# templeblock/llzlab

Hardware: AMD Instinct MI355X
Metric: Msamples/s/GPU (float32 FIR 257-tap, 4096 ch) + achieved HBM GB/s vs peak (higher is better)
Workload: dtype f32; 1 GPU; 4096-ch float32 FIR, 257 taps (llz_fir_lpf_cof 0.1 KAISER), 1048576 samples/ch per GPU, overlap-save-1024, channels sharded over 1 GPU(s); channels_per_gpu=4096, samples_per_channel=1048576, taps=257, algorithm=overlap-save-1024

## Files before the change

### llzlab_amd/csrc/kernels/fft32.hpp

```cpp
#pragma once
#include "common.hpp"

namespace {

struct cf {
    float x, y;
};

__device__ __forceinline__ cf cadd(cf a, cf b) { return {a.x + b.x, a.y + b.y}; }
__device__ __forceinline__ cf csub(cf a, cf b) { return {a.x - b.x, a.y - b.y}; }

template <bool CONJ>
__device__ __forceinline__ cf cmul(cf a, cf w)
{
    if (CONJ) return {__builtin_fmaf(a.y, w.y, a.x * w.x), __builtin_fmaf(-a.x, w.y, a.y * w.x)};
    return {__builtin_fmaf(-a.y, w.y, a.x * w.x), __builtin_fmaf(a.x, w.y, a.y * w.x)};
}

__device__ constexpr float kCos32[9] = {1.0f, 0.98078528040323044913f, 0.92387953251128675613f,
                                        0.83146961230254523708f, 0.70710678118654752440f,
                                        0.55557023301960222474f, 0.38268343236508977173f,
                                        0.19509032201612826785f, 0.0f};

template <bool INV>
__device__ __forceinline__ cf tw32(cf d, int q)
{
    if (q == 0) return d;
    if (q == 8) return INV ? cf{-d.y, d.x} : cf{d.y, -d.x};
    constexpr float r = 0.70710678118654752440f;
    if (q == 4) return INV ? cf{(d.x - d.y) * r, (d.x + d.y) * r} : cf{(d.x + d.y) * r, (d.y - d.x) * r};
    if (q == 12) return INV ? cf{-(d.x + d.y) * r, (d.x - d.y) * r} : cf{(d.y - d.x) * r, -(d.x + d.y) * r};
    const float c = q <= 8 ? kCos32[q] : -kCos32[16 - q];
    const float s = q <= 8 ? kCos32[8 - q] : kCos32[q - 8];
    return cmul<!INV>(d, cf{c, s});
}

__device__ constexpr int brev5(int r)
{
    return ((r & 1) << 4) | ((r & 2) << 2) | (r & 4) | ((r & 8) >> 2) | ((r & 16) >> 4);
}

#ifndef LLZ_OLS_DIT
#define LLZ_OLS_DIT 1
#endif

#if !LLZ_OLS_DIT
template <bool INV>
__device__ __forceinline__ void fft32(cf (&v)[32])
{
#pragma unroll
    for (int span = 32; span >= 2; span >>= 1) {
        const int half = span >> 1;
        const int tstep = 32 / span;
#pragma unroll
        for (int blk = 0; blk < 32; blk += span) {
#pragma unroll
            for (int q = 0; q < half; q++) {
                const cf a = v[blk + q], b = v[blk + q + half];
                v[blk + q] = cadd(a, b);
                v[blk + q + half] = tw32<INV>(csub(a, b), q * tstep);
            }
        }
    }
}
#else
template <bool INV>
__device__ __forceinline__ void bfly_dit(cf &a, cf &b, int q)
{
    const cf A = a, B = b;
    if (q == 0) {
        a = cadd(A, B); b = csub(A, B);
        return;
    }
    if (q == 8) {
        const cf wb = INV ? cf{-B.y, B.x} : cf{B.y, -B.x};
        a = cadd(A, wb); b = csub(A, wb);
        return;
    }
    const float c = q <= 8 ? kCos32[q] : -kCos32[16 - q];
    const float s0 = q <= 8 ? kCos32[8 - q] : kCos32[q - 8];
    const float s = INV ? s0 : -s0;
    float p, g, f;
    if (c >= s0 || -c >= s0) {
        const float t = s / c;
        p = __builtin_fmaf(-t, B.y, B.x);
        g = __builtin_fmaf(t, B.x, B.y);
        f = c;
    } else {
        const float r = c / s;
        p = __builtin_fmaf(-r, B.x, B.y);
        g = __builtin_fmaf(r, B.y, B.x);
        a = cf{__builtin_fmaf(-s, p, A.x), __builtin_fmaf(s, g, A.y)};
        b = cf{__builtin_fmaf(s, p, A.x), __builtin_fmaf(-s, g, A.y)};
        return;
    }
    a = cf{__builtin_fmaf(f, p, A.x), __builtin_fmaf(f, g, A.y)};
    b = cf{__builtin_fmaf(-f, p, A.x), __builtin_fmaf(-f, g, A.y)};
}

template <bool INV>
__device__ __forceinline__ void fft32(cf (&v)[32])
{
    cf w[32];
#pragma unroll
    for (int i = 0; i < 32; i++) w[i] = v[brev5(i)];
#pragma unroll
    for (int half = 1; half <= 16; half <<= 1) {
        const int tstep = 16 / half;
#pragma unroll
        for (int blk = 0; blk < 32; blk += 2 * half) {
#pragma unroll
            for (int q = 0; q < half; q++) bfly_dit<INV>(w[blk + q], w[blk + q + half], q * tstep);
        }
    }
#pragma unroll
    for (int r = 0; r < 32; r++) v[r] = w[brev5(r)];
}
#endif

constexpr int OLS_PITCH = 33;
constexpr int OLS_XBUF = 32 * OLS_PITCH;
__device__ __forceinline__ int xaddr(int row, int col) { return row * OLS_PITCH + col; }

#define OLS_WAVE_SYNC() asm volatile("s_waitcnt lgkmcnt(0)" ::: "memory")

template <bool INV>
__device__ __forceinline__ void transpose_twiddle(cf (&v)[32], float *buf, const float2 *__restrict__ tw, int wcol, int rrow)
{
#pragma unroll
    for (int r = 0; r < 32; r++) {
        const float2 w = tw[brev5(r) * 32 + wcol];
        v[r] = cmul<INV>(v[r], cf{w.x, w.y});
    }
#pragma unroll
    for (int r = 0; r < 32; r++) buf[xaddr(brev5(r), wcol)] = v[r].x;
    OLS_WAVE_SYNC();
#pragma unroll
    for (int cidx = 0; cidx < 32; cidx++) v[cidx].x = buf[xaddr(rrow, cidx)];
    OLS_WAVE_SYNC();
#pragma unroll
    for (int r = 0; r < 32; r++) buf[xaddr(brev5(r), wcol)] = v[r].y;
    OLS_WAVE_SYNC();
#pragma unroll
    for (int cidx = 0; cidx < 32; cidx++) v[cidx].y = buf[xaddr(rrow, cidx)];
    OLS_WAVE_SYNC();
}

template <bool INV>
__device__ __forceinline__ void transpose_twiddle(cf (&v)[32], float *buf, const float2 *__restrict__ tw, int l5)
{
    transpose_twiddle<INV>(v, buf, tw, l5, l5);
}

__device__ __forceinline__ void swap32(float &x, float &y)
{
    const auto p = __builtin_amdgcn_permlane32_swap(__float_as_uint(x), __float_as_uint(y), false, false);
    x = __uint_as_float(p[0]);
    y = __uint_as_float(p[1]);
}

}
```

### llzlab_amd/csrc/kernels/fir_ols.hip

```cpp
#include <stdlib.h>
#include "common.hpp"
#include "fft32.hpp"

namespace {

constexpr int OLS_N = 1024;
constexpr int OLS_OVERLAP = 256;
constexpr int OLS_VALID = OLS_N - OLS_OVERLAP;
constexpr int OLS_JOB = 2 * OLS_VALID;
constexpr int OLS_WAVES = 4;
constexpr int OLS_THREADS = 64 * OLS_WAVES;
constexpr int OLS_SEG = 16;

struct ols_lane {
    int half, col;
};

__device__ __forceinline__ ols_lane ols_lane_of(int lane)
{
    ols_lane g;
    g.half = lane >> 5;
    g.col = lane & 31;
    return g;
}

struct ols_seg {
    bool live;
    int c, j0, count;
};

struct ols_geom {
    int n, keep, jobs_per_channel, segs_per_channel, seg_len;
    long total_segs, in_pitch, out_pitch;
};

__device__ __forceinline__ ols_seg ols_locate(long seg, const ols_geom &G)
{
    ols_seg g;
    g.live = seg < G.total_segs;
    g.c = g.live ? (int)(seg / G.segs_per_channel) : 0;
    g.j0 = g.live ? (int)(seg - (long)g.c * G.segs_per_channel) * G.seg_len : 0;
    g.count = g.live ? min(G.seg_len, G.jobs_per_channel - g.j0) : 0;
    return g;
}

struct ols_raw {
    float a[24], b[24];
};

__device__ __forceinline__ void ols_load(ols_raw &raw, const float *const (&row)[2], const int (&s)[2],
                                         const bool (&live)[2], const ols_lane &g, int n)
{
    const bool whole = live[0] && live[1] && s[0] + OLS_JOB <= n && s[1] + OLS_JOB <= n;
    const float *r = g.half ? row[1] : row[0];
    const int so = g.half ? s[1] : s[0];
    const bool lv = g.half ? live[1] : live[0];
    if (whole) {
#pragma unroll
        for (int i = 0; i < 24; i++) {
            raw.a[i] = __builtin_nontemporal_load(&r[so + 32 * i + g.col]);
            raw.b[i] = __builtin_nontemporal_load(&r[so + OLS_VALID + 32 * i + g.col]);
        }
    } else {
#pragma unroll
        for (int i = 0; i < 24; i++) {
            const int ia = so + 32 * i + g.col, ib = ia + OLS_VALID;
            const float xa = r[min(ia, n - 1)], xb = r[min(ib, n - 1)];
            raw.a[i] = (lv && ia < n) ? xa : 0.f;
            raw.b[i] = (lv && ib < n) ? xb : 0.f;
        }
    }
}

__device__ __forceinline__ void ols_load_halo(float (&halo)[8], const float *row, const float *hrow, int s, int col,
                                              int keep, bool live)
{
#pragma unroll
    for (int i = 0; i < 8; i++) {
        const int idx = s - OLS_OVERLAP + 32 * i + col;
        float v = 0.f;
        if (live) {
            if (idx >= 0) v = row[idx];
            else if (hrow && idx >= -keep) v = hrow[keep + idx];
        }
        halo[i] = v;
    }
}

__device__ __forceinline__ void ols_filter(cf (&v)[32], cf (&u)[32], float *buf, const float2 *s_tw,
                                           const float2 *s_h, int l5, int col)
{
    fft32<false>(v);
    transpose_twiddle<false>(v, buf, s_tw, col, l5);
    fft32<false>(v);
#pragma unroll
    for (int r = 0; r < 32; r++) {
        const float2 h = s_h[l5 + 32 * brev5(r)];
        u[brev5(r)] = cmul<false>(v[r], cf{h.x, h.y});
    }
    fft32<true>(u);
    transpose_twiddle<true>(u, buf, s_tw, l5, col);
    fft32<true>(u);
}

__device__ __forceinline__ void ols_store(const cf (&u)[32], float *const (&orow)[2], const int (&s)[2],
                                          const bool (&live)[2], const ols_lane &g, int n)
{
    const bool whole = live[0] && live[1] && s[0] + OLS_JOB <= n && s[1] + OLS_JOB <= n;
    const bool lv = g.half ? live[1] : live[0];
    if (!lv) return;
    float *o = g.half ? orow[1] : orow[0];
    const int so = g.half ? s[1] : s[0];
    const int oa = so + g.col - OLS_OVERLAP;
    const int ob = oa + OLS_VALID;
    if (whole) {
#pragma unroll
        for (int r = 0; r < 32; r++) {
            const int n1 = brev5(r);
            if (n1 >= 8) {
                __builtin_nontemporal_store(u[r].x, &o[oa + 32 * n1]);
                __builtin_nontemporal_store(u[r].y, &o[ob + 32 * n1]);
            }
        }
    } else {
#pragma unroll
        for (int r = 0; r < 32; r++) {
            const int n1 = brev5(r);
            if (n1 >= 8) {
                if (oa + 32 * n1 < n) o[oa + 32 * n1] = u[r].x;
                if (ob + 32 * n1 < n) o[ob + 32 * n1] = u[r].y;
            }
        }
    }
}

__device__ __forceinline__ void ols_assemble(cf (&v)[32], float (&halo)[8], const ols_raw &raw)
{
#pragma unroll
    for (int i = 0; i < 8; i++) {
        v[i].x = halo[i];
        v[i].y = raw.a[16 + i];
        halo[i] = raw.b[16 + i];
    }
#pragma unroll
    for (int i = 0; i < 24; i++) {
        v[8 + i].x = raw.a[i];
        v[8 + i].y = raw.b[i];
    }
}

struct ols_smem {
    float2 *tw, *h;
    float *buf;
};

__device__ __forceinline__ ols_smem ols_tables(char *smem, const float2 *__restrict__ hfreq, const float2 *__restrict__ twid)
{
    ols_smem m;
    m.tw = reinterpret_cast<float2 *>(smem);
    m.h = m.tw + 1024;
    for (int i = threadIdx.x; i < 1024; i += OLS_THREADS) {
        m.tw[i] = twid[i];
        m.h[i] = hfreq[i];
    }
    __syncthreads();
    const int wave = threadIdx.x >> 6, half = (threadIdx.x >> 5) & 1;
    m.buf = reinterpret_cast<float *>(m.h + 1024) + (wave * 2 + half) * OLS_XBUF;
    return m;
}

__global__ void __launch_bounds__(OLS_THREADS, 2)
k_fir_ols_chain_f32(const float *__restrict__ in, float *__restrict__ out, const float *__restrict__ hist,
                    const float2 *__restrict__ hfreq, const float2 *__restrict__ twid, ols_geom G)
{
    extern __shared__ __attribute__((aligned(16))) char smem[];
    const ols_smem S = ols_tables(smem, hfreq, twid);
    const int lane = threadIdx.x & 63;
    const int wave = __builtin_amdgcn_readfirstlane(threadIdx.x >> 6);
    const int l5 = lane & 31;
    const ols_lane g = ols_lane_of(lane);
    const long halves_total = (long)gridDim.x * OLS_WAVES * 2;
    const long first = ((long)blockIdx.x * OLS_WAVES + wave) * 2;

    ols_seg cur[2] = {ols_locate(first, G), ols_locate(first + 1, G)};
    float halo[8];
    ols_raw raw;
    {
        const float *const row[2] = {in + (size_t)cur[0].c * G.in_pitch, in + (size_t)cur[1].c * G.in_pitch};
        const ols_seg own = g.half ? cur[1] : cur[0];
        ols_load_halo(halo, g.half ? row[1] : row[0], hist ? hist + (size_t)own.c * G.keep : nullptr, own.j0 * OLS_JOB,
                      g.col, G.keep, own.live);
        const int s0[2] = {cur[0].j0 * OLS_JOB, cur[1].j0 * OLS_JOB};
        const bool lv[2] = {cur[0].count > 0, cur[1].count > 0};
        ols_load(raw, row, s0, lv, g, G.n);
    }
    for (long sp = first; sp < G.total_segs; sp += halves_total) {
        const ols_seg nxt[2] = {ols_locate(sp + halves_total, G), ols_locate(sp + halves_total + 1, G)};
        const float *const row[2] = {in + (size_t)cur[0].c * G.in_pitch, in + (size_t)cur[1].c * G.in_pitch};
        float *const orow[2] = {out + (size_t)cur[0].c * G.out_pitch, out + (size_t)cur[1].c * G.out_pitch};
        const float *const nrow[2] = {in + (size_t)nxt[0].c * G.in_pitch, in + (size_t)nxt[1].c * G.in_pitch};
        const ols_seg nown = g.half ? nxt[1] : nxt[0];
        float halo_n[8];
#pragma unroll
        for (int i = 0; i < 8; i++) halo_n[i] = 0.f;

        const int jmax = max(cur[0].count, cur[1].count);
#pragma unroll 1
        for (int jj = 0; jj < jmax; jj++) {
            const int s[2] = {(cur[0].j0 + jj) * OLS_JOB, (cur[1].j0 + jj) * OLS_JOB};
            const bool live[2] = {jj < cur[0].count, jj < cur[1].count};
            cf v[32], u[32];
            ols_assemble(v, halo, raw);
            const bool in_pair = jj + 1 < jmax;
            {
                const float *const lrow[2] = {in_pair ? row[0] : nrow[0], in_pair ? row[1] : nrow[1]};
                const int sn[2] = {in_pair ? s[0] + OLS_JOB : nxt[0].j0 * OLS_JOB,
                                   in_pair ? s[1] + OLS_JOB : nxt[1].j0 * OLS_JOB};
                const bool ln[2] = {in_pair ? jj + 1 < cur[0].count : nxt[0].count > 0,
                                    in_pair ? jj + 1 < cur[1].count : nxt[1].count > 0};
                ols_load(raw, lrow, sn, ln, g, G.n);
            }
            if (!in_pair)
                ols_load_halo(halo_n, g.half ? nrow[1] : nrow[0], hist ? hist + (size_t)nown.c * G.keep : nullptr,
                              nown.j0 * OLS_JOB, g.col, G.keep, nown.live);
            ols_filter(v, u, S.buf, S.tw, S.h, l5, g.col);
            ols_store(u, orow, s, live, g, G.n);
        }
        cur[0] = nxt[0];
        cur[1] = nxt[1];
#pragma unroll
        for (int i = 0; i < 8; i++) halo[i] = halo_n[i];
    }
}



template <int O>
__global__ void __launch_bounds__(OLS_THREADS, 2)
k_fir_ols2k_chain_f32(const float *__restrict__ in, float *__restrict__ out, const float *__restrict__ hist,
                     const float2 *__restrict__ hfreq2 ,
                     const float2 *__restrict__ twid , const float2 *__restrict__ tw2k ,
                     ols_geom G)
{
    extern __shared__ __attribute__((aligned(16))) char smem[];
    float2 *s_tw = reinterpret_cast<float2 *>(smem);
    float2 *s_h = s_tw + 1024;
    float2 *s_w = s_h + 2048;
    for (int i = threadIdx.x; i < 1024; i += OLS_THREADS) {
        s_tw[i] = twid[i];
        s_h[i] = hfreq2[i];
        s_h[1024 + i] = hfreq2[1024 + i];
        s_w[i] = tw2k[i];
    }
    __syncthreads();
    constexpr int O2K_OVERLAP = O, O2K_VALID = 2048 - O, O2K_JOB = 2 * O2K_VALID;
    constexpr int HP = O / 64, NEW = 32 - HP;
    const int lane = threadIdx.x & 63;
    const int wave = __builtin_amdgcn_readfirstlane(threadIdx.x >> 6);
    const int half = lane >> 5, l5 = lane & 31;
    float *buf = reinterpret_cast<float *>(s_w + 1024) + (wave * 2 + half) * OLS_XBUF;
    const float2 *my_h = s_h + half * 1024;
    const long waves_total = (long)gridDim.x * OLS_WAVES;
    const int rowoff = 32 * half + l5;

    struct segd { const float *row; float *orow; const float *hrow; int j0, count; };
    auto locate = [&](long seg) {
        segd d;
        const bool live = seg < G.total_segs;
        const int c = live ? (int)(seg / G.segs_per_channel) : 0;
        d.j0 = live ? (int)(seg - (long)c * G.segs_per_channel) * G.seg_len : 0;
        d.count = live ? min(G.seg_len, G.jobs_per_channel - d.j0) : 0;
        d.row = in + (size_t)c * G.in_pitch;
        d.orow = out + (size_t)c * G.out_pitch;
        d.hrow = hist ? hist + (size_t)c * G.keep : nullptr;
        return d;
    };
    const int n = G.n;
    auto load_halo = [&](float (&halo)[HP], const segd &d) {
#pragma unroll
        for (int i = 0; i < HP; i++) {
            const int idx = d.j0 * O2K_JOB - O2K_OVERLAP + 64 * i + rowoff;
            float v = 0.f;
            if (d.count > 0) {
                if (idx >= 0) v = d.row[idx];
                else if (d.hrow && idx >= -G.keep) v = d.hrow[G.keep + idx];
            }
            halo[i] = v;
        }
    };
    ols_raw raw;
    auto load = [&](const float *row, int s, bool live) {
        if (live && s + O2K_JOB <= n) {
#pragma unroll
            for (int i = 0; i < NEW; i++) {
                raw.a[i] = __builtin_nontemporal_load(&row[s + 64 * i + rowoff]);
                raw.b[i] = __builtin_nontemporal_load(&row[s + O2K_VALID + 64 * i + rowoff]);
            }
        } else {
#pragma unroll
            for (int i = 0; i < NEW; i++) {
                const int ia = s + 64 * i + rowoff, ib = ia + O2K_VALID;
                const float xa = row[min(ia, n - 1)], xb = row[min(ib, n - 1)];
                raw.a[i] = (live && ia < n) ? xa : 0.f;
                raw.b[i] = (live && ib < n) ? xb : 0.f;
            }
        }
    };

    long seg = (long)blockIdx.x * OLS_WAVES + wave;
    segd cur = locate(seg);
    float halo[HP];
    load_halo(halo, cur);
    load(cur.row, cur.j0 * O2K_JOB, cur.count > 0);
    for (; seg < G.total_segs; seg += waves_total) {
        const segd nxt = locate(seg + waves_total);
        float halo_n[HP];
#pragma unroll
        for (int i = 0; i < HP; i++) halo_n[i] = 0.f;
#pragma unroll 1
        for (int jj = 0; jj < cur.count; jj++) {
            const int s = (cur.j0 + jj) * O2K_JOB;
            const float *row = cur.row;
            float *orow = cur.orow;
            cf v[32], u[32];
#pragma unroll
            for (int i = 0; i < HP; i++) {
                v[i].x = halo[i];
                v[i].y = raw.a[NEW - HP + i];
                halo[i] = raw.b[NEW - HP + i];
            }
#pragma unroll
            for (int i = 0; i < NEW; i++) {
                v[HP + i].x = raw.a[i];
                v[HP + i].y = raw.b[i];
            }
            const bool in_seg = jj + 1 < cur.count;
            load(in_seg ? row : nxt.row, in_seg ? s + O2K_JOB : nxt.j0 * O2K_JOB, in_seg || nxt.count > 0);
            if (!in_seg) load_halo(halo_n, nxt);
            cf w[32];
#pragma unroll
            for (int p = 0; p < 16; p++) {
                cf sm = cadd(v[p], v[p + 16]);
                const float2 t = s_w[64 * p + rowoff];
                cf df = cmul<false>(csub(v[p], v[p + 16]), cf{t.x, t.y});
                swap32(sm.x, df.x);
                swap32(sm.y, df.y);
                w[2 * p] = sm;
                w[2 * p + 1] = df;
            }
            ols_filter(w, u, buf, s_tw, my_h, l5, l5);
            const bool whole = s + O2K_JOB <= n;
            const int oa = s - O2K_OVERLAP + rowoff, ob = oa + O2K_VALID;
#pragma unroll
            for (int p = 0; p < 16; p++) {
                cf P = u[brev5(2 * p)], Q = u[brev5(2 * p + 1)];
                swap32(P.x, Q.x);
                swap32(P.y, Q.y);
                const float2 t = s_w[64 * p + rowoff];
                Q = cmul<true>(Q, cf{t.x, t.y});
                const cf y0 = cadd(P, Q), y1 = csub(P, Q);
                if (whole) {
                    if (p >= HP) {
                        __builtin_nontemporal_store(y0.x, &orow[oa + 64 * p]);
                        __builtin_nontemporal_store(y0.y, &orow[ob + 64 * p]);
                    }
                    __builtin_nontemporal_store(y1.x, &orow[oa + 64 * (p + 16)]);
                    __builtin_nontemporal_store(y1.y, &orow[ob + 64 * (p + 16)]);
                } else {
                    if (p >= HP) {
                        if (oa + 64 * p < n) orow[oa + 64 * p] = y0.x;
                        if (ob + 64 * p < n) orow[ob + 64 * p] = y0.y;
                    }
                    if (oa + 64 * (p + 16) < n) orow[oa + 64 * (p + 16)] = y1.x;
                    if (ob + 64 * (p + 16) < n) orow[ob + 64 * (p + 16)] = y1.y;
                }
            }
        }
        cur = nxt;
#pragma unroll
        for (int i = 0; i < HP; i++) halo[i] = halo_n[i];
    }
}


__device__ __forceinline__ int o8k_lane()
{
    int l = (int)__builtin_amdgcn_mbcnt_hi(~0u, __builtin_amdgcn_mbcnt_lo(~0u, 0u));
    asm volatile("" : "+v"(l));
    return l;
}
constexpr int O4K_WAVES = 8, O4K_THREADS = 64 * O4K_WAVES;

template <int WS = 1>
__device__ __forceinline__ void ols2k_core(cf (&v)[32], cf (&y)[32], float *buf, const float2 *s_tw, const float2 *my_h,
                                           const float2 *s_w, int l5, int rowoff)
{
    cf w[32], u[32];
#pragma unroll
    for (int p = 0; p < 16; p++) {
        cf sm = cadd(v[p], v[p + 16]);
        const float2 t = s_w[WS * (64 * p + rowoff)];
        cf df = cmul<false>(csub(v[p], v[p + 16]), cf{t.x, t.y});
        swap32(sm.x, df.x);
        swap32(sm.y, df.y);
        w[2 * p] = sm;
        w[2 * p + 1] = df;
    }
    ols_filter(w, u, buf, s_tw, my_h, l5, l5);
#pragma unroll
    for (int p = 0; p < 16; p++) {
        cf P = u[brev5(2 * p)], Q = u[brev5(2 * p + 1)];
        swap32(P.x, Q.x);
        swap32(P.y, Q.y);
        const float2 t = s_w[WS * (64 * p + rowoff)];
        Q = cmul<true>(Q, cf{t.x, t.y});
        y[p] = cadd(P, Q);
        y[p + 16] = csub(P, Q);
    }
}

template <int O>
__global__ void __launch_bounds__(O4K_THREADS, 2)
k_fir_ols4k_f32(const float *__restrict__ in, float *__restrict__ out, const float *__restrict__ hist,
                const float2 *__restrict__ hfreq4 , const float2 *__restrict__ twid ,
                const float2 *__restrict__ tw2k , const float2 *__restrict__ tw4k ,
                ols_geom G)
{
    constexpr int V = 4096 - O, JOB = 2 * V, PO = O / 64, PV = V / 64;
    extern __shared__ __attribute__((aligned(16))) char smem[];
    float2 *s_tw = reinterpret_cast<float2 *>(smem);
    float2 *s_w2 = s_tw + 1024;
    float2 *s_w4 = s_w2 + 1024;
    float2 *s_h = s_w4 + 2048;
    for (int i = threadIdx.x; i < 1024; i += O4K_THREADS) {
        s_tw[i] = twid[i];
        s_w2[i] = tw2k[i];
        s_w4[i] = tw4k[i];
        s_w4[1024 + i] = tw4k[1024 + i];
#pragma unroll
        for (int j = 0; j < 4; j++) s_h[1024 * j + i] = hfreq4[1024 * j + i];
    }
    __syncthreads();
    const int wave = __builtin_amdgcn_readfirstlane(threadIdx.x >> 6);
    float *s_buf = reinterpret_cast<float *>(s_h + 4096);
    const long waves_total = (long)gridDim.x * O4K_WAVES;
    const int n = G.n;

    for (long seg = (long)blockIdx.x * O4K_WAVES + wave; seg < G.total_segs; seg += waves_total) {
        const int c = (int)(seg / G.segs_per_channel);
        const int j0 = (int)(seg - (long)c * G.segs_per_channel) * G.seg_len;
        const int count = min(G.seg_len, G.jobs_per_channel - j0);
        const float *row = in + (size_t)c * G.in_pitch;
        float *orow = out + (size_t)c * G.out_pitch;
        const float *hrow = hist ? hist + (size_t)c * G.keep : nullptr;
#pragma unroll 1
        for (int jj = 0; jj < count; jj++) {
            const int s = (j0 + jj) * JOB;
            cf v[64];
            const bool whole = s >= O && s + JOB <= n;
            {
            const int rowoff = o8k_lane();
            if (whole) {
#pragma unroll
                for (int i = 0; i < PO; i++) v[i].x = row[s - O + 64 * i + rowoff];
#pragma unroll
                for (int i = PO; i < 64; i++) v[i].x = __builtin_nontemporal_load(&row[s - O + 64 * i + rowoff]);
#pragma unroll
                for (int i = PO; i < 64; i++) v[i].y = __builtin_nontemporal_load(&row[s + V - O + 64 * i + rowoff]);
            } else {
#pragma unroll
                for (int i = 0; i < 64; i++) {
                    const int ia = s - O + 64 * i + rowoff;
                    float xa = 0.f;
                    if (ia >= 0) xa = row[min(ia, n - 1)];
                    else if (hrow && ia >= -G.keep) xa = hrow[G.keep + ia];
                    v[i].x = ia < n ? xa : 0.f;
                }
#pragma unroll
                for (int i = PO; i < 64; i++) {
                    const int ib = s + V - O + 64 * i + rowoff;
                    const float xb = row[min(ib, n - 1)];
                    v[i].y = ib < n ? xb : 0.f;
                }
            }
            }
#pragma unroll
            for (int i = 0; i < PO; i++) v[i].y = v[i + PV].x;
            const int rowoff = o8k_lane(), half = rowoff >> 5, l5 = rowoff & 31;
            float *buf = s_buf + (wave * 2 + half) * OLS_XBUF;
            cf e[32], o[32];
#pragma unroll
            for (int p = 0; p < 32; p++) {
                e[p] = cadd(v[p], v[p + 32]);
                const float2 t = s_w4[64 * p + rowoff];
                o[p] = cmul<false>(csub(v[p], v[p + 32]), cf{t.x, t.y});
            }
            cf ye[32], yo[32];
            ols2k_core(e, ye, buf, s_tw, s_h + (2 * half) * 1024, s_w2, l5, rowoff);
            ols2k_core(o, yo, buf, s_tw, s_h + (2 * half + 1) * 1024, s_w2, l5, rowoff);
            const bool all_out = s + JOB <= n;
#pragma unroll
            for (int p = 0; p < 32; p++) {
                if (p + 32 < PO) continue;
                const float2 t = s_w4[64 * p + rowoff];
                const cf q = cmul<true>(yo[p], cf{t.x, t.y});
                if (p >= PO) {
                    const cf y0 = cadd(ye[p], q);
                    const int oa = s + 64 * (p - PO) + rowoff, ob = oa + V;
                    if (all_out) {
                        __builtin_nontemporal_store(y0.x, &orow[oa]);
                        __builtin_nontemporal_store(y0.y, &orow[ob]);
                    } else {
                        if (oa < n) orow[oa] = y0.x;
                        if (ob < n) orow[ob] = y0.y;
                    }
                }
                const cf y1 = csub(ye[p], q);
                const int oa = s + 64 * (p + 32 - PO) + rowoff, ob = oa + V;
                if (all_out) {
                    __builtin_nontemporal_store(y1.x, &orow[oa]);
                    __builtin_nontemporal_store(y1.y, &orow[ob]);
                } else {
                    if (oa < n) orow[oa] = y1.x;
                    if (ob < n) orow[ob] = y1.y;
                }
            }
        }
    }
}


#ifdef O8K_TRACE
__device__ unsigned long long o8k_trace_buf[2048 * 8];
#define O8K_T0() unsigned long long o8_t = __builtin_readcyclecounter(), o8_acc[8] = {0, 0, 0, 0, 0, 0, 0, 0}
#define O8K_MARK(i) do { const unsigned long long now = __builtin_readcyclecounter(); o8_acc[i] += now - o8_t; o8_t = now; } while (0)
#define O8K_PIN(x) asm volatile("s_nop 0" ::"v"(x))
#define O8K_DUMP() do { if ((threadIdx.x & 63) == 0) { const unsigned wv_ = (blockIdx.x * (blockDim.x >> 6) + (threadIdx.x >> 6)) & 2047u; \
    for (int i = 0; i < 8; i++) o8k_trace_buf[wv_ * 8 + i] = o8_acc[i]; } } while (0)
#else
#define O8K_T0() do { } while (0)
#define O8K_MARK(i) do { } while (0)
#define O8K_PIN(x) do { } while (0)
#define O8K_DUMP() do { } while (0)
#endif
struct w128_tab {
    float c[64], s[64];
};
constexpr double o8k_sin(double x)
{
    double term = x, sum = x;
    for (int k = 1; k < 16; k++) {
        term *= -x * x / (double)((2 * k) * (2 * k + 1));
        sum += term;
    }
    return sum;
}
constexpr double o8k_cos(double x)
{
    double term = 1.0, sum = 1.0;
    for (int k = 1; k < 16; k++) {
        term *= -x * x / (double)((2 * k - 1) * (2 * k));
        sum += term;
    }
    return sum;
}
constexpr w128_tab o8k_make_w128()
{
    w128_tab t{};
    for (int j = 0; j < 64; j++) {
        const double a = 3.14159265358979323846 * (double)j / 64.0;
        t.c[j] = j == 32 ? 0.f : (float)o8k_cos(a);
        t.s[j] = j == 0 ? 0.f : (float)o8k_sin(a);
    }
    return t;
}
__device__ constexpr w128_tab kW128 = o8k_make_w128();

constexpr int O8K_WAVES = 8, O8K_THREADS = 64 * O8K_WAVES, O8K_PAIRS = O8K_WAVES / 2;
#ifndef O8K_SPIN
#define O8K_SPIN (1 << 18)
#endif
constexpr int O8K_SPIN_LIMIT = O8K_SPIN;

typedef __attribute__((address_space(3))) volatile int *o8k_flag_p;
typedef float o8k_f2 __attribute__((ext_vector_type(2)));
typedef __attribute__((address_space(3))) o8k_f2 *o8k_box_p;
struct o8k_pair {
    o8k_flag_p my_free, my_sent, pt_free, pt_sent;
    o8k_box_p my_box, pt_box;
    int k;
};
__device__ __forceinline__ void o8k_signal(o8k_flag_p flag, int k)
{
    asm volatile("s_waitcnt lgkmcnt(0)" ::: "memory");
    *flag = k;
}
__device__ __forceinline__ void o8k_wait(o8k_flag_p flag, int k)
{
    int spins = 0;
    while (__builtin_amdgcn_readfirstlane(*flag) < k && ++spins < O8K_SPIN_LIMIT) __builtin_amdgcn_s_sleep(1);
    asm volatile("" ::: "memory");
}
template <int OFF>
__device__ __forceinline__ void o8k_swap(cf (&a)[64], o8k_pair &ps)
{
    const int lane = o8k_lane();
    const o8k_box_p mine = ps.my_box + lane, theirs = ps.pt_box + lane;
#pragma unroll
    for (int r = 0; r < 2; r++) {
        ps.k++;
        o8k_signal(ps.my_free, ps.k);
        o8k_wait(ps.pt_free, ps.k);
#pragma unroll
        for (int i = 0; i < 16; i++) theirs[64 * i] = (o8k_f2){a[OFF + 16 * r + i].x, a[OFF + 16 * r + i].y};
        o8k_signal(ps.my_sent, ps.k);
        o8k_wait(ps.pt_sent, ps.k);
#pragma unroll
        for (int i = 0; i < 16; i++) {
            const o8k_f2 t = mine[64 * i];
            a[OFF + 16 * r + i] = cf{t[0], t[1]};
        }
    }
    asm volatile("s_waitcnt lgkmcnt(0)" ::: "memory");
}

__device__ __forceinline__ void ols4k_core(cf (&a)[64], float *buf, const float2 *s_tw, const float2 *s_w4, const float2 *h_e,
                                           const float2 *h_o, int l5, int rowoff)
{
    cf e[32], o[32];
#pragma unroll
    for (int p = 0; p < 32; p++) {
        e[p] = cadd(a[p], a[p + 32]);
        const float2 t = s_w4[64 * p + rowoff];
        o[p] = cmul<false>(csub(a[p], a[p + 32]), cf{t.x, t.y});
    }
    cf ye[32], yo[32];
    ols2k_core<2>(e, ye, buf, s_tw, h_e, s_w4, l5, rowoff);
    ols2k_core<2>(o, yo, buf, s_tw, h_o, s_w4, l5, rowoff);
#pragma unroll
    for (int p = 0; p < 32; p++) {
        const float2 t = s_w4[64 * p + rowoff];
        const cf q = cmul<true>(yo[p], cf{t.x, t.y});
        a[p] = cadd(ye[p], q);
        a[p + 32] = csub(ye[p], q);
    }
}

template <int O>
__global__ void __launch_bounds__(O8K_THREADS, 2)
k_fir_ols8k_f32(const float *__restrict__ in, float *__restrict__ out, const float *__restrict__ hist,
                const float2 *__restrict__ hfreq8 , const float2 *__restrict__ twid ,
                const float2 *__restrict__ tw4k , ols_geom G)
{
    constexpr int V = 8192 - O, JOB = 2 * V, PO = O / 64;
    static_assert(O % 64 == 0 && O <= 6144, "at least 2048 new samples per block");
    extern __shared__ __attribute__((aligned(16))) char smem[];
    float2 *s_tw = reinterpret_cast<float2 *>(smem);
    float2 *s_w4 = s_tw + 1024;
    float2 *s_h = s_w4 + 2048;
    float *s_buf = reinterpret_cast<float *>(s_h + 8192);
    int *s_flag = reinterpret_cast<int *>(s_buf + 2 * O8K_WAVES * OLS_XBUF);
    float2 *s_wl = reinterpret_cast<float2 *>(s_flag + 2 * O8K_WAVES);
    for (int i = threadIdx.x; i < 1024; i += O8K_THREADS) {
        s_tw[i] = twid[i];
        s_w4[i] = tw4k[i];
        s_w4[1024 + i] = tw4k[1024 + i];
#pragma unroll
        for (int j = 0; j < 8; j++) s_h[1024 * j + i] = hfreq8[1024 * j + i];
    }
    if (threadIdx.x < 2 * O8K_WAVES) s_flag[threadIdx.x] = 0;
    if (threadIdx.x < 64) {
        float sn, cs;
        sincospif((float)threadIdx.x * (1.0f / 4096.0f), &sn, &cs);
        s_wl[threadIdx.x] = make_float2(cs, -sn);
    }
    __syncthreads();
    const int wave = __builtin_amdgcn_readfirstlane(threadIdx.x >> 6);
#ifdef O8K_CROSS_SIMD
    const int w = wave & 1, pair = wave >> 1, partner = wave ^ 1;
#else
    const int w = wave >> 2, pair = wave & 3, partner = wave ^ 4;
#endif
    o8k_pair ps;
    ps.my_free = (o8k_flag_p)(s_flag + 2 * wave);
    ps.my_sent = (o8k_flag_p)(s_flag + 2 * wave + 1);
    ps.pt_free = (o8k_flag_p)(s_flag + 2 * partner);
    ps.pt_sent = (o8k_flag_p)(s_flag + 2 * partner + 1);
    ps.my_box = (o8k_box_p)(reinterpret_cast<o8k_f2 *>(s_buf + (wave * 2) * OLS_XBUF));
    ps.pt_box = (o8k_box_p)(reinterpret_cast<o8k_f2 *>(s_buf + (partner * 2) * OLS_XBUF));
    ps.k = 0;
    O8K_T0();
    const long pairs_total = (long)gridDim.x * O8K_PAIRS;
    const int n = G.n;
    const int pos0 = 32 * w;

    for (long seg = (long)blockIdx.x * O8K_PAIRS + pair; seg < G.total_segs; seg += pairs_total) {
        const int c = (int)(seg / G.segs_per_channel);
        const int j0 = (int)(seg - (long)c * G.segs_per_channel) * G.seg_len;
        const int count = min(G.seg_len, G.jobs_per_channel - j0);
        const float *row = in + (size_t)c * G.in_pitch;
        float *orow = out + (size_t)c * G.out_pitch;
        const float *hrow = hist ? hist + (size_t)c * G.keep : nullptr;
#pragma unroll 1
        for (int jj = 0; jj < count; jj++) {
            const int s = (j0 + jj) * JOB;
            O8K_MARK(6);
            cf a[64];
            const bool whole = s >= O && s + JOB <= n;
            if (whole) {
                const float *ra = row + s - O + 64 * pos0 + o8k_lane(), *rb = ra + V;
#pragma unroll
                for (int j = 0; j < 32; j++) {
                    a[j].x = __builtin_nontemporal_load(&ra[64 * j]);
                    a[32 + j].x = __builtin_nontemporal_load(&ra[64 * (j + 64)]);
                }
#pragma unroll
                for (int j = 0; j < 32; j++) {
                    a[j].y = __builtin_nontemporal_load(&rb[64 * j]);
                    a[32 + j].y = __builtin_nontemporal_load(&rb[64 * (j + 64)]);
                }
            } else {
                const int lane = o8k_lane();
#pragma unroll
                for (int j = 0; j < 64; j++) {
                    const int pos = pos0 + (j < 32 ? j : j + 32);
                    const int ia = s - O + 64 * pos + lane, ib = ia + V;
                    float xa = 0.f;
                    if (ia >= 0) xa = row[min(ia, n - 1)];
                    else if (hrow && ia >= -G.keep) xa = hrow[G.keep + ia];
                    a[j].x = ia < n ? xa : 0.f;
                    float xb;
                    if (O > 4096 && ib < 0) xb = (hrow && ib >= -G.keep) ? hrow[G.keep + ib] : 0.f;
                    else xb = row[min(ib, n - 1)];
                    a[j].y = ib < n ? xb : 0.f;
                }
            }
            O8K_PIN(a[0].x); O8K_PIN(a[63].y); O8K_PIN(a[31].y); O8K_PIN(a[32].x);
            O8K_MARK(0);
            const float2 wd = s_wl[o8k_lane()];
            const cf wv = w ? cf{wd.y, -wd.x} : cf{wd.x, wd.y};
#pragma unroll
            for (int j = 0; j < 32; j++) {
                const cf sm = cadd(a[j], a[32 + j]), df = csub(a[j], a[32 + j]);
                const cf t = cmul<false>(cf{kW128.c[j], -kW128.s[j]}, wv);
                const cf dt = cmul<false>(df, t);
                a[j] = w ? dt : sm;
                a[32 + j] = w ? sm : dt;
            }
            O8K_PIN(a[0].x); O8K_PIN(a[63].y);
            O8K_MARK(1);
            o8k_swap<32>(a, ps);
            O8K_PIN(a[32].x); O8K_PIN(a[63].y);
            O8K_MARK(2);
            {
                const int ln = o8k_lane(), hf = ln >> 5;
                ols4k_core(a, s_buf + (wave * 2 + hf) * OLS_XBUF, s_tw, s_w4, s_h + (4 * hf + w) * 1024, s_h + (4 * hf + 2 + w) * 1024,
                           ln & 31, ln);
            }
            O8K_PIN(a[0].x); O8K_PIN(a[63].y); O8K_PIN(a[32].x);
            O8K_MARK(3);
            if (w) {
                const float2 wr = s_wl[o8k_lane()];
                const cf wu = cf{wr.x, wr.y};
#pragma unroll
                for (int p = 0; p < 64; p++) {
                    const cf t = cmul<false>(cf{kW128.c[p ^ 32], -kW128.s[p ^ 32]}, wu);
                    a[p] = cmul<true>(a[p], t);
                }
            }
            o8k_swap<32>(a, ps);
            O8K_PIN(a[32].x); O8K_PIN(a[63].y); O8K_PIN(a[0].x);
            O8K_MARK(4);
            const float sg = w ? -1.f : 1.f;
            const int lane = o8k_lane();
            const bool all_out = s + JOB <= n;
            const int jmin = PO - pos0;
            float *oa0 = orow + s + 64 * (pos0 - PO) + lane;
#pragma unroll
            for (int j = 0; j < 32; j++) {
                const cf y0 = cadd(a[j], a[32 + j]), d1 = csub(a[j], a[32 + j]);
                const cf y1 = cf{d1.x * sg, d1.y * sg};
                const int oa = s + 64 * (pos0 + j - PO) + lane, ob = oa + V;
                if (all_out) {
                    if (j >= jmin) {
                        __builtin_nontemporal_store(y0.x, &oa0[64 * j]);
                        __builtin_nontemporal_store(y0.y, &oa0[64 * j + V]);
                    }
                    if (PO <= 64 || j >= jmin - 64) {
                        __builtin_nontemporal_store(y1.x, &oa0[64 * (j + 64)]);
                        __builtin_nontemporal_store(y1.y, &oa0[64 * (j + 64) + V]);
                    }
                } else {
                    if (j >= jmin) {
                        if (oa < n) orow[oa] = y0.x;
                        if (ob < n) orow[ob] = y0.y;
                    }
                    if (PO <= 64 || j >= jmin - 64) {
                        if (oa + 4096 < n) orow[oa + 4096] = y1.x;
                        if (ob + 4096 < n) orow[ob + 4096] = y1.y;
                    }
                }
            }
            O8K_MARK(5);
#ifdef O8K_TRACE
            o8_acc[7]++;
#endif
        }
    }
    O8K_DUMP();
}


struct ols_rung {
    int nfft, min_taps;
    const char *name;
    int threads;
    int segs_per_wg;
    int wg_per_cu;
    bool tuned;
    double startup;
    size_t lds_bytes;
    bool w2k, w4k;
    int count;
    int overlap[8];
    const void *kernel[8];
};

template <typename K> static const void *kfn(K k) { return reinterpret_cast<const void *>(k); }

const ols_rung OLS_RUNGS[] = {
    {1024, 1, "k_fir_ols_f32", OLS_THREADS, 2 * OLS_WAVES, 2, true, 1.0,
     2 * 1024 * sizeof(float2) + (size_t)OLS_WAVES * 2 * OLS_XBUF * sizeof(float), false, false,
     1, {OLS_OVERLAP}, {kfn(k_fir_ols_chain_f32)}},
    {2048, 2, "k_fir_ols2k_chain_f32", OLS_THREADS, OLS_WAVES, 2, false, 1.0,
     4 * 1024 * sizeof(float2) + (size_t)OLS_WAVES * 2 * OLS_XBUF * sizeof(float), true, false,
     2, {512, 1024}, {kfn(k_fir_ols2k_chain_f32<512>), kfn(k_fir_ols2k_chain_f32<1024>)}},
    {4096, 2, "k_fir_ols4k_f32", O4K_THREADS, O4K_WAVES, 1, false, 0.0,
     8 * 1024 * sizeof(float2) + (size_t)O4K_WAVES * 2 * OLS_XBUF * sizeof(float), true, true,
     7, {512, 768, 1024, 1536, 2048, 2560, 3072},
     {kfn(k_fir_ols4k_f32<512>), kfn(k_fir_ols4k_f32<768>), kfn(k_fir_ols4k_f32<1024>), kfn(k_fir_ols4k_f32<1536>),
      kfn(k_fir_ols4k_f32<2048>), kfn(k_fir_ols4k_f32<2560>), kfn(k_fir_ols4k_f32<3072>)}},
    {8192, 2, "k_fir_ols8k_f32", O8K_THREADS, O8K_PAIRS, 1, false, 0.0,
     (1024 + 2048 + 8192) * sizeof(float2) + (size_t)O8K_WAVES * 2 * OLS_XBUF * sizeof(float) + 2 * O8K_WAVES * sizeof(int) +
         64 * sizeof(float2), false, true,
     8, {1536, 2304, 2560, 3072, 3584, 4096, 5120, 6144},
     {kfn(k_fir_ols8k_f32<1536>), kfn(k_fir_ols8k_f32<2304>), kfn(k_fir_ols8k_f32<2560>), kfn(k_fir_ols8k_f32<3072>),
      kfn(k_fir_ols8k_f32<3584>), kfn(k_fir_ols8k_f32<4096>), kfn(k_fir_ols8k_f32<5120>), kfn(k_fir_ols8k_f32<6144>)}},
};

struct ols_plan {
    int instance;
    long blocks;
    ols_geom G;
};

static ols_plan ols_plan_of(const ols_rung &r, int channels, int n, long in_pitch, long out_pitch, int flt_len)
{
    ols_plan p;
    p.instance = 0;
    while (r.overlap[p.instance] < flt_len - 1) p.instance++;
    const int job = 2 * (r.nfft - r.overlap[p.instance]);
    ols_geom &G = p.G;
    G.n = n;
    G.keep = flt_len - 1;
    G.in_pitch = in_pitch;
    G.out_pitch = out_pitch;
    G.jobs_per_channel = (n + job - 1) / job;
    const int tuned_per_cu = r.tuned ? llzs_tune(LLZS_TUNE_OLS_WG_PER_CU) : -1;
    const long max_blocks = 256L * (tuned_per_cu > 0 ? tuned_per_cu : r.wg_per_cu);
    const long slots = max_blocks * r.segs_per_wg;
    int seg_len = OLS_SEG;
    if ((long)((G.jobs_per_channel + OLS_SEG - 1) / OLS_SEG) * channels < 4 * slots) {
        double best = 1e300;
        for (int sl = OLS_SEG; sl >= 1; sl--) {
            const long segs = (long)((G.jobs_per_channel + sl - 1) / sl) * channels;
            const double cost = (double)((segs + slots - 1) / slots) * (sl + r.startup);
            if (cost < best * 0.999) { best = cost; seg_len = sl; }
        }
    }
    if (r.tuned)
        if (const int v = llzs_tune(LLZS_TUNE_OLS_SEG_LEN); v >= 1 && v <= 1024) seg_len = v;
    G.seg_len = seg_len;
    G.segs_per_channel = (G.jobs_per_channel + seg_len - 1) / seg_len;
    G.total_segs = (long)G.segs_per_channel * channels;
    p.blocks = (G.total_segs + r.segs_per_wg - 1) / r.segs_per_wg;
    if (p.blocks > max_blocks) p.blocks = max_blocks;
    return p;
}

}

extern "C" int llzs_fir_ols_f32(int nfft, const llzs_ols_tables *t, const float *in, float *out, const float *hist, int channels,
                                int n, long in_pitch, long out_pitch, int flt_len, void *stream)
{
    const ols_rung *r = nullptr;
    for (const ols_rung &c : OLS_RUNGS)
        if (c.nfft == nfft) r = &c;
    if (!r || !t || !t->hfreq || !t->twid || (r->w2k && !t->tw2k) || (r->w4k && !t->tw4k) || !in || !out || channels <= 0 ||
        n <= 0 || in_pitch < n || out_pitch < n) {
        llzs_set_error("fir_ols_f32: bad arguments (%d points)", nfft);
        return LLZ_ERR_ARG;
    }
    if (flt_len < r->min_taps || flt_len - 1 > r->overlap[r->count - 1]) {
        llzs_set_error("fir_ols_f32: flt_len %d outside %d..%d (%d points)", flt_len, r->min_taps, r->overlap[r->count - 1] + 1,
                       nfft);
        return LLZ_ERR_RANGE;
    }
    ols_plan p = ols_plan_of(*r, channels, n, in_pitch, out_pitch, flt_len);
    const float2 *hf = reinterpret_cast<const float2 *>(t->hfreq), *tw = reinterpret_cast<const float2 *>(t->twid),
                 *w2 = reinterpret_cast<const float2 *>(t->tw2k), *w4 = reinterpret_cast<const float2 *>(t->tw4k);
    void *args[8] = {&in, &out, &hist, &hf, &tw};
    int k = 5;
    if (r->w2k) args[k++] = &w2;
    if (r->w4k) args[k++] = &w4;
    args[k] = &p.G;
    const void *kernel = r->kernel[p.instance];
    if (r->lds_bytes > 64 * 1024)
        LLZ_HIP_CHECK(hipFuncSetAttribute(kernel, hipFuncAttributeMaxDynamicSharedMemorySize, (int)r->lds_bytes));
    (void)hipLaunchKernel(kernel, dim3((unsigned)p.blocks), dim3(r->threads), args, r->lds_bytes, as_stream(stream));
    LLZ_LAUNCH_CHECK(r->name);
    return LLZ_OK;
}

#ifdef O8K_TRACE
extern "C" int llzs_o8k_trace_read(unsigned long long *dst, int count)
{
    LLZ_HIP_CHECK(hipDeviceSynchronize());
    LLZ_HIP_CHECK(hipMemcpyFromSymbol(dst, HIP_SYMBOL(o8k_trace_buf), sizeof(unsigned long long) * (size_t)count));
    return LLZ_OK;
}
#endif
```

Baseline: 662,200 Msamples/s.

## Cut register pressure in OLS-1024 kernel and balance segment partitioning

Rewrites the 1024-point OLS filter to run in place with a single 32-element complex array. It uses grouped FFT32 butterflies pinned with empty asm, double-buffered twiddle and filter table products, and halo reload straight into the live halo buffer. Scheduling barriers are added in the tail load loop. Occupancy is raised to 3 workgroups per CU, and segments are now split evenly per channel with a remainder distribution instead of fixed-length segments. The aim is less VGPR use for higher occupancy and better load balance, at the risk of spills or worse instruction scheduling under the asm constraints.

```diff
diff --git a/llzlab_amd/csrc/kernels/fft32.hpp b/llzlab_amd/csrc/kernels/fft32.hpp
--- a/llzlab_amd/csrc/kernels/fft32.hpp
+++ b/llzlab_amd/csrc/kernels/fft32.hpp
@@ -116,6 +116,43 @@
 #pragma unroll
     for (int r = 0; r < 32; r++) v[r] = w[brev5(r)];
 }
+
+constexpr int FFT32_GRP = 4;
+__device__ __forceinline__ void fft32_pin(cf &c) { asm volatile("" : "+v"(c.x), "+v"(c.y)); }
+
+template <bool INV>
+__device__ __forceinline__ void fft32_grouped(cf (&v)[32])
+{
+    cf w[32];
+#pragma unroll
+    for (int i = 0; i < 32; i++) w[i] = v[brev5(i)];
+#pragma unroll
+    for (int half = 1; half <= 16; half <<= 1) {
+        const int tstep = 16 / half;
+#pragma unroll
+        for (int b0 = 0; b0 < 16; b0 += FFT32_GRP) {
+#pragma unroll
+            for (int b = b0; b < b0 + FFT32_GRP && half > 1; b++) {
+                const int lo = (b / half) * 2 * half + b % half;
+                fft32_pin(w[lo]);
+                fft32_pin(w[lo + half]);
+            }
+#pragma unroll
+            for (int b = b0; b < b0 + FFT32_GRP; b++) {
+                const int lo = (b / half) * 2 * half + b % half;
+                bfly_dit<INV>(w[lo], w[lo + half], (b % half) * tstep);
+            }
+#pragma unroll
+            for (int b = b0; b < b0 + FFT32_GRP; b++) {
+                const int lo = (b / half) * 2 * half + b % half;
+                fft32_pin(w[lo]);
+                fft32_pin(w[lo + half]);
+            }
+        }
+    }
+#pragma unroll
+    for (int r = 0; r < 32; r++) v[r] = w[brev5(r)];
+}
 #endif
 
 constexpr int OLS_PITCH = 33;
diff --git a/llzlab_amd/csrc/kernels/fir_ols.hip b/llzlab_amd/csrc/kernels/fir_ols.hip
--- a/llzlab_amd/csrc/kernels/fir_ols.hip
+++ b/llzlab_amd/csrc/kernels/fir_ols.hip
@@ -30,7 +30,7 @@
 };
 
 struct ols_geom {
-    int n, keep, jobs_per_channel, segs_per_channel, seg_len;
+    int n, keep, jobs_per_channel, segs_per_channel, seg_len, seg_extra;
     long total_segs, in_pitch, out_pitch;
 };
 
@@ -39,8 +39,9 @@
     ols_seg g;
     g.live = seg < G.total_segs;
     g.c = g.live ? (int)(seg / G.segs_per_channel) : 0;
-    g.j0 = g.live ? (int)(seg - (long)g.c * G.segs_per_channel) * G.seg_len : 0;
-    g.count = g.live ? min(G.seg_len, G.jobs_per_channel - g.j0) : 0;
+    const int k = g.live ? (int)(seg - (long)g.c * G.segs_per_channel) : 0;
+    g.j0 = k * G.seg_len + min(k, G.seg_extra);
+    g.count = g.live ? G.seg_len + (k < G.seg_extra ? 1 : 0) : 0;
     return g;
 }
 
@@ -68,6 +69,7 @@
             const float xa = r[min(ia, n - 1)], xb = r[min(ib, n - 1)];
             raw.a[i] = (lv && ia < n) ? xa : 0.f;
             raw.b[i] = (lv && ib < n) ? xb : 0.f;
+            if (i % 4 == 3) __builtin_amdgcn_sched_barrier(0);
         }
     }
 }
@@ -101,6 +103,64 @@
     fft32<true>(u);
     transpose_twiddle<true>(u, buf, s_tw, l5, col);
     fft32<true>(u);
+}
+
+constexpr int OLS_GRP = 2;
+
+template <bool CONJ, typename IDX>
+__device__ __forceinline__ void ols_table_product(cf (&v)[32], const float2 *tab, IDX idx)
+{
+    float2 w[2][OLS_GRP];
+#pragma unroll
+    for (int i = 0; i < OLS_GRP; i++) w[0][i] = tab[idx(i)];
+#pragma unroll
+    for (int g = 0; g < 32 / OLS_GRP; g++) {
+        if (g + 1 < 32 / OLS_GRP) {
+#pragma unroll
+            for (int i = 0; i < OLS_GRP; i++) w[(g + 1) & 1][i] = tab[idx((g + 1) * OLS_GRP + i)];
+        }
+#pragma unroll
+        for (int i = 0; i < OLS_GRP; i++) {
+            const int r = g * OLS_GRP + i;
+            v[r] = cmul<CONJ>(v[r], cf{w[g & 1][i].x, w[g & 1][i].y});
+            asm volatile("" : "+v"(v[r].x), "+v"(v[r].y) : : "memory");
+        }
+    }
+}
+
+template <bool INV>
+__device__ __forceinline__ void ols_transpose_twiddle(cf (&v)[32], float *buf, const float2 *tw, int wcol, int rrow)
+{
+    ols_table_product<INV>(v, tw, [=](int r) { return brev5(r) * 32 + wcol; });
+#pragma unroll
+    for (int r = 0; r < 32; r++) buf[xaddr(brev5(r), wcol)] = v[r].x;
+    OLS_WAVE_SYNC();
+#pragma unroll
+    for (int cidx = 0; cidx < 32; cidx++) v[cidx].x = buf[xaddr(rrow, cidx)];
+    OLS_WAVE_SYNC();
+#pragma unroll
+    for (int r = 0; r < 32; r++) buf[xaddr(brev5(r), wcol)] = v[r].y;
+    OLS_WAVE_SYNC();
+#pragma unroll
+    for (int cidx = 0; cidx < 32; cidx++) v[cidx].y = buf[xaddr(rrow, cidx)];
+    OLS_WAVE_SYNC();
+}
+
+__device__ __forceinline__ void ols_filter_inplace(cf (&v)[32], float *buf, const float2 *s_tw, const float2 *s_h, int l5,
+                                                   int col)
+{
+    fft32_grouped<false>(v);
+    ols_transpose_twiddle<false>(v, buf, s_tw, col, l5);
+    fft32_grouped<false>(v);
+    ols_table_product<false>(v, s_h, [=](int r) { return l5 + 32 * brev5(r); });
+    cf u[32];
+#pragma unroll
+    for (int r = 0; r < 32; r++) u[brev5(r)] = v[r];
+    fft32_grouped<true>(u);
+    ols_transpose_twiddle<true>(u, buf, s_tw, l5, col);
+    fft32_grouped<true>(u);
+#pragma unroll
+    for (int r = 0; r < 32; r++) v[r] = u[r];
 }
 
 __device__ __forceinline__ void ols_store(const cf (&u)[32], float *const (&orow)[2], const int (&s)[2],
@@ -169,7 +229,7 @@
     return m;
 }
 
-__global__ void __launch_bounds__(OLS_THREADS, 2)
+__global__ void __launch_bounds__(OLS_THREADS, 3)
 k_fir_ols_chain_f32(const float *__restrict__ in, float *__restrict__ out, const float *__restrict__ hist,
                     const float2 *__restrict__ hfreq, const float2 *__restrict__ twid, ols_geom G)
 {
@@ -199,17 +259,13 @@
         const float *const row[2] = {in + (size_t)cur[0].c * G.in_pitch, in + (size_t)cur[1].c * G.in_pitch};
         float *const orow[2] = {out + (size_t)cur[0].c * G.out_pitch, out + (size_t)cur[1].c * G.out_pitch};
         const float *const nrow[2] = {in + (size_t)nxt[0].c * G.in_pitch, in + (size_t)nxt[1].c * G.in_pitch};
-        const ols_seg nown = g.half ? nxt[1] : nxt[0];
-        float halo_n[8];
-#pragma unroll
-        for (int i = 0; i < 8; i++) halo_n[i] = 0.f;
 
         const int jmax = max(cur[0].count, cur[1].count);
 #pragma unroll 1
         for (int jj = 0; jj < jmax; jj++) {
             const int s[2] = {(cur[0].j0 + jj) * OLS_JOB, (cur[1].j0 + jj) * OLS_JOB};
             const bool live[2] = {jj < cur[0].count, jj < cur[1].count};
-            cf v[32], u[32];
+            cf v[32];
             ols_assemble(v, halo, raw);
             const bool in_pair = jj + 1 < jmax;
             {
@@ -220,16 +276,18 @@
                                     in_pair ? jj + 1 < cur[1].count : nxt[1].count > 0};
                 ols_load(raw, lrow, sn, ln, g, G.n);
             }
-            if (!in_pair)
-                ols_load_halo(halo_n, g.half ? nrow[1] : nrow[0], hist ? hist + (size_t)nown.c * G.keep : nullptr,
-                              nown.j0 * OLS_JOB, g.col, G.keep, nown.live);
-            ols_filter(v, u, S.buf, S.tw, S.h, l5, g.col);
-            ols_store(u, orow, s, live, g, G.n);
+            if (!in_pair) {
+                int col = g.col, half = g.half;
+                asm volatile("" : "+v"(col), "+v"(half));
+                const ols_seg nown = half ? nxt[1] : nxt[0];
+                ols_load_halo(halo, half ? nrow[1] : nrow[0], hist ? hist + (size_t)nown.c * G.keep : nullptr,
+                              nown.j0 * OLS_JOB, col, G.keep, nown.live);
+            }
+            ols_filter_inplace(v, S.buf, S.tw, S.h, l5, g.col);
+            ols_store(v, orow, s, live, g, G.n);
         }
         cur[0] = nxt[0];
         cur[1] = nxt[1];
-#pragma unroll
-        for (int i = 0; i < 8; i++) halo[i] = halo_n[i];
     }
 }
 
@@ -829,7 +887,7 @@
 template <typename K> static const void *kfn(K k) { return reinterpret_cast<const void *>(k); }
 
 const ols_rung OLS_RUNGS[] = {
-    {1024, 1, "k_fir_ols_f32", OLS_THREADS, 2 * OLS_WAVES, 2, true, 1.0,
+    {1024, 1, "k_fir_ols_f32", OLS_THREADS, 2 * OLS_WAVES, 3, true, 1.0,
      2 * 1024 * sizeof(float2) + (size_t)OLS_WAVES * 2 * OLS_XBUF * sizeof(float), false, false,
      1, {OLS_OVERLAP}, {kfn(k_fir_ols_chain_f32)}},
     {2048, 2, "k_fir_ols2k_chain_f32", OLS_THREADS, OLS_WAVES, 2, false, 1.0,
@@ -870,18 +928,29 @@
     const long max_blocks = 256L * (tuned_per_cu > 0 ? tuned_per_cu : r.wg_per_cu);
     const long slots = max_blocks * r.segs_per_wg;
     int seg_len = OLS_SEG;
-    if ((long)((G.jobs_per_channel + OLS_SEG - 1) / OLS_SEG) * channels < 4 * slots) {
+    const int min_segs = (G.jobs_per_channel + OLS_SEG - 1) / OLS_SEG;
+    int segs = min_segs;
+    if ((long)min_segs * channels < 4 * slots) {
         double best = 1e300;
         for (int sl = OLS_SEG; sl >= 1; sl--) {
-            const long segs = (long)((G.jobs_per_channel + sl - 1) / sl) * channels;
-            const double cost = (double)((segs + slots - 1) / slots) * (sl + r.startup);
+            const long total = (long)((G.jobs_per_channel + sl - 1) / sl) * channels;
+            const double cost = (double)((total + slots - 1) / slots) * (sl + r.startup);
             if (cost < best * 0.999) { best = cost; seg_len = sl; }
         }
+        segs = (G.jobs_per_channel + seg_len - 1) / seg_len;
+    } else if (r.tuned) {
+        double best = 1e300;
+        for (int sc = min_segs; sc <= G.jobs_per_channel && sc <= 2 * min_segs; sc++) {
+            const long rounds = ((long)sc * channels + slots - 1) / slots;
+            const double cost = (double)rounds * ((double)G.jobs_per_channel / sc + r.startup);
+            if (cost < best * 0.999) { best = cost; segs = sc; }
+        }
     }
     if (r.tuned)
-        if (const int v = llzs_tune(LLZS_TUNE_OLS_SEG_LEN); v >= 1 && v <= 1024) seg_len = v;
-    G.seg_len = seg_len;
-    G.segs_per_channel = (G.jobs_per_channel + seg_len - 1) / seg_len;
+        if (const int v = llzs_tune(LLZS_TUNE_OLS_SEG_LEN); v >= 1 && v <= 1024) segs = (G.jobs_per_channel + v - 1) / v;
+    G.segs_per_channel = segs;
+    G.seg_len = r.tuned ? G.jobs_per_channel / segs : seg_len;
+    G.seg_extra = r.tuned ? G.jobs_per_channel % segs : 0;
     G.total_segs = (long)G.segs_per_channel * channels;
     p.blocks = (G.total_segs + r.segs_per_wg - 1) / r.segs_per_wg;
     if (p.blocks > max_blocks) p.blocks = max_blocks;
```

After: 610,400 Msamples/s. -7.8%, worse.
